# gmarcais/Jellyfish

Measured on AMD Instinct MI355X. Metric: k-mers/sec at k=21 canonical, 150 bp synthetic reads, bit-exact counts, higher is better.
Workload: dtype u64

## Files before the change

### jellyfish_amd/csrc/jfgpu.hip

```cpp
#include <hip/hip_runtime.h>
#include <math.h>
#include <stdint.h>
#include <stdio.h>
#include <string.h>
#include <algorithm>
#include <memory>
#include <string>
#include <type_traits>
#include <vector>

#include "../../include/jfgpu.h"
#include "gf2_matrix.hpp"
#include "tuning.hpp"
#include "kernels.hip.hpp"
#include "kernels_part.hip.hpp"
#include "kernels_tile.hip.hpp"
#include "kernels_p1ring.hip.hpp"
#include "kernels_bloom.hip.hpp"
#include "kernels_bloom_part.hip.hpp"
#include "kernels_wide.hip.hpp"
#include "kernels_wide_part.hip.hpp"
#include "kernels_nword.hip.hpp"
#include "kernels_parse.hip.hpp"
#include "kernels_bgzf.hip.hpp"
// ... 783 lines not shown
    HIP_TRY(hipFuncSetAttribute((const void*)tile_insert_wide_kernel<true>, hipFuncAttributeMaxDynamicSharedMemorySize, wt));
    HIP_TRY(hipFuncSetAttribute((const void*)tile_insert_wide_kernel<false>, hipFuncAttributeMaxDynamicSharedMemorySize, wt));
    HIP_TRY(hipFuncSetAttribute((const void*)tile_insert_wide_pipe_kernel<true>, hipFuncAttributeMaxDynamicSharedMemorySize, wt));
    HIP_TRY(hipFuncSetAttribute((const void*)tile_insert_wide_pipe_kernel<false>, hipFuncAttributeMaxDynamicSharedMemorySize, wt));
  }
  jfgpu_table* raw = t.release();
  int rc = jfgpu_clear(raw);
  if(rc) { jfgpu_destroy(raw); return rc; }
  *out = raw;
  return JFGPU_OK;
}

void jfgpu_destroy(jfgpu_table* t) {
  if(!t) return;
  hipSetDevice(t->device);
  if(t->stream) hipStreamSynchronize(t->stream);
  prof_collect(t);
  for(auto e : t->ev_pool) hipEventDestroy(e);
  hipFree(t->dt.slots); hipFree(t->d_fwd); hipFree(t->d_inv);
  if(t->d_dt) hipFree(t->d_dt);
  hipFree(t->dt.ovf_key); hipFree(t->dt.ovf_cnt); hipFree(t->dt.counters); hipFree(t->dt.dirty);
  for(int i = 0; i < 2; ++i) { if(t->d_stage[i]) hipFree(t->d_stage[i]); if(t->stage_done[i]) hipEventDestroy(t->stage_done[i]); }
  if(t->d_dump) hipFree(t->d_dump);
  if(t->d_bcache) hipFree(t->d_bcache);
  if(t->d_tile_off) hipFree(t->d_tile_off);
  part_discard(t);
  if(t->d_M1) hipFree(t->d_M1);
  if(t->d_strag) hipFree(t->d_strag);
  if(t->d_strag2) hipFree(t->d_strag2);
  if(t->d_strag2_n) hipFree(t->d_strag2_n);
  if(t->d_strag_n) hipFree(t->d_strag_n);
  if(t->d_M2) hipFree(t->d_M2);
  if(t->ws) hipFree(t->ws);
  if(t->stream2) hipStreamDestroy(t->stream2);
  for(auto ev : t->flush_ev) if(ev) hipEventDestroy(ev);
  if(t->flush_done) hipEventDestroy(t->flush_done);
  if(t->stream) hipStreamDestroy(t->stream);
  delete t;
}

int jfgpu_get_info(const jfgpu_table* t, jfgpu_info* o) {
  if(!t || !o) return fail(JFGPU_E_INVALID, "null argument");
  memset(o, 0, sizeof(*o));
  o->k = t->g.k; o->key_len = t->g.key_bits; o->canonical = t->g.canonical;
  o->lsize = t->g.lsize_g; o->size = 1ull << t->g.lsize_g; o->local_size = 1ull << t->g.lsize_l;
  o->shard_bits = t->g.shard_bits; o->shard_id = t->g.shard_id;
  o->val_len = t->g.cnt_bits; o->slot_bytes = (uint32_t)slot_bytes_of(t); o->tile_slots = 1u << t->g.tile_bits;
  o->matrix_identity = t->matrix.identity ? 1 : 0;
  o->out_counter_len = t->out_counter_len;
  o->max_reprobe = t->dt.max_probe;
  o->table_bytes = (1ull << t->g.lsize_l) * slot_bytes_of(t);
  return JFGPU_OK;
}

int jfgpu_get_matrix(const jfgpu_table* t, uint64_t* columns) {
  if(!t || !columns) return fail(JFGPU_E_INVALID, "null argument");
  memcpy(columns, t->matrix.columns.data(), sizeof(uint64_t) * t->matrix.c);
  return JFGPU_OK;
}

int jfgpu_clear(jfgpu_table* t) {
  if(t) { t->failed = 0; t->failed_msg.clear(); }
  int rc = use(t); if(rc) return rc;
  part_discard(t);
  HIP_TRY(hipMemsetAsync(t->dt.slots, 0, (1ull << t->g.lsize_l) * slot_bytes_of(t), t->stream));
  HIP_TRY(hipMemsetAsync(t->dt.ovf_key, 0, t->ovf_cap * sizeof(uint64_t), t->stream));
  HIP_TRY(hipMemsetAsync(t->dt.ovf_cnt, 0, t->ovf_cap * sizeof(uint64_t), t->stream));
  HIP_TRY(hipMemsetAsync(t->dt.counters, 0, CTR_COUNT * sizeof(uint64_t), t->stream));
  HIP_TRY(hipMemsetAsync(t->dt.dirty, 0, (size_t)1 << (t->g.lsize_l - t->g.tile_bits), t->stream));
  HIP_TRY(hipStreamSynchronize(t->stream));
  t->pristine = true; t->occ_known = 0; t->fed_since = 0; t->direct_seen = 0; t->occ_bound = 0; t->bigval_bound = 0; t->ovf_failed_need = 0;
  t->flushes_plain = 0; t->flushes_heavy = 0;
  t->n_p2_roles = t->n_p2_ring = t->n_p2_sort = t->n_p2_exact = t->n_p1_ring = t->n_p1_other = t->n_tile_dense = 0;
  return JFGPU_OK;
}

int jfgpu_sync(jfgpu_table* t) {
  int rc = use(t); if(rc) return rc;
  rc = part_flush(t); if(rc) return rc;
  HIP_TRY(hipStreamSynchronize(t->stream));
#ifdef JFGPU_PHASE_PROF
  { unsigned long long c[24], z[24] = {0};
    if(hipMemcpyFromSymbol(c, HIP_SYMBOL(g_phase_prof), sizeof c) == hipSuccess) {
      fprintf(stderr, "[phase prof] P1 (ring): stage %llu  encode+hash+append %llu  (barrier) %llu  units out %llu  finish %llu\n",
              c[0], c[1], c[2], c[3], c[4]);
      fprintf(stderr, "[phase prof] P2: (barrier) %llu  load %llu  hist %llu  scan %llu  lds-scatter %llu  write-out %llu  finish %llu\n",
              c[8], c[9], c[10], c[11], c[12], c[13], c[14]);
      fprintf(stderr, "[phase prof] T: loop+offsets %llu  rank adds + fill %llu  place %llu  merge %llu  queue (wave 0's own) %llu  (its wait for the others) %llu  store %llu\n",
              c[16], c[17], c[18], c[22], c[21], c[19], c[20]);
      (void)hipMemcpyToSymbol(HIP_SYMBOL(g_phase_prof), z, sizeof z);
    } }
#endif
#ifdef JFGPU_TILE_PROF
  { uint64_t c[CTR_COUNT]; if(read_counters(t, c) == JFGPU_OK)
      fprintf(stderr, "[tile prof] wait+prefetch %llu  fill %llu  insert %llu  store %llu (shader clocks, summed over blocks)\n",
              (unsigned long long)c[CTR_PROF0], (unsigned long long)c[CTR_PROF0 + 1], (unsigned long long)c[CTR_PROF0 + 2], (unsigned long long)c[CTR_PROF0 + 3]); }
#endif
  return check_deferred(t);
}

int jfgpu_wait(jfgpu_table* t) {
  int rc = use(t); if(rc) return rc;
  HIP_TRY(hipStreamSynchronize(t->stream));
  return JFGPU_OK;
}

int jfgpu_count_ascii_dev(jfgpu_table* t, const char* d_bases, size_t n) {
  int rc = use(t); if(rc) return rc;
  if(t->g.shard_bits) return fail(JFGPU_E_INVALID, "sharded table: count through its communicator (jfgpu_comm_count_ascii_dev)");
  if(!d_bases && n) return fail(JFGPU_E_INVALID, "null buffer");
  return launch_count(t, d_bases, n);
}

int jfgpu_count_ascii(jfgpu_table* t, const char* bases, size_t n) {
  int rc = use(t); if(rc) return rc;
  if(t->g.shard_bits) return fail(JFGPU_E_INVALID, "sharded table: count through its communicator (jfgpu_comm_count_ascii_dev)");
  if(!bases && n) return fail(JFGPU_E_INVALID, "null buffer");
  if(n < t->g.k) return JFGPU_OK;
  rc = ensure_stage(t); if(rc) return rc;
  const size_t step = kStageBytes - (t->g.k - 1);
  for(size_t o = 0; o < n; o += step) {
    const size_t len = std::min(kStageBytes, n - o);
    const int b = t->stage_next; t->stage_next ^= 1;
    HIP_TRY(hipEventSynchronize(t->stage_done[b]));
    HIP_TRY(hipMemcpyAsync(t->d_stage[b], bases + o, len, hipMemcpyHostToDevice, t->stream));
    rc = launch_count(t, (const char*)t->d_stage[b], len); if(rc) return rc;
    HIP_TRY(hipEventRecord(t->stage_done[b], t->stream));
    if(o + len >= n) break;
  }
  return JFGPU_OK;
}

static int add_keys_piece(jfgpu_table* t, const uint64_t* d_keys, size_t n, uint64_t val, uint8_t* d_is_new) {
  int rc = JFGPU_OK;
  if(!n) return JFGPU_OK;
  { const bool big = t->g.cnt_bits < 64 && (val >> t->g.cnt_bits) != 0;
    rc = ensure_ovf(t, big ? 0 : (uint64_t)n * val, big ? n : 0); if(rc) return rc; }
  const bool one_word = !t->wide && !t->nword;
  if(one_word && val == 1 && !d_is_new && use_partitioned(t, n * 8)) {
    const int prc = part_ingest(t, (const uint8_t*)d_keys, 0, (int64_t)n, true, n);
    if(prc >= 0) return prc;
  }
  if(one_word && (d_is_new || val != 1)) { rc = part_flush(t); if(rc) return rc; }
  if(!t->wide) t->pristine = false;
  const int grid = grid_for(t, (n + kBlock - 1) / kBlock);
  ProfScope ps(t, 1, n);
  if(one_word && val == 1 && !d_is_new) {
    if(t->returning) hipLaunchKernelGGL(add_keys_one_kernel<true>, dim3(grid), dim3(kBlock), 0, t->stream, t->dt, d_keys, (uint64_t)n);
    else             hipLaunchKernelGGL(add_keys_one_kernel<false>, dim3(grid), dim3(kBlock), 0, t->stream, t->dt, d_keys, (uint64_t)n);
  } else {
    with_view(t, [&](const auto& T) {
      hipLaunchKernelGGL(add_keys_kernel, dim3(grid), dim3(kBlock), 0, t->stream, T, d_keys, (uint64_t)n, t->key_words, val, d_is_new);
    });
  }
  HIP_TRY(hipGetLastError());
  return JFGPU_OK;
}

int jfgpu_add_keys_dev(jfgpu_table* t, const uint64_t* d_keys, size_t n, uint64_t val, uint8_t* d_is_new) {
  int rc = use(t); if(rc) return rc;
  if(!n) return JFGPU_OK;
  if(!d_keys) return fail(JFGPU_E_INVALID, "null keys");
  if(!capacity_managed(t)) return add_keys_piece(t, d_keys, n, val, d_is_new);
  size_t off = 0;
  while(off < n) {
    uint64_t take = 0;
    rc = ensure_capacity(t, n - off, &take); if(rc) return rc;
    rc = add_keys_piece(t, d_keys + off * t->key_words, (size_t)take, val, d_is_new ? d_is_new + off : nullptr); if(rc) return rc;
    off += (size_t)take;
  }
  return JFGPU_OK;
}

// ... 395 lines not shown
```

### jellyfish_amd/csrc/kernels.hip.hpp

```cpp
#pragma once
#include <hip/hip_runtime.h>
#include <stdint.h>
#include "kmer_core.hpp"

namespace jfgpu {

constexpr int kBlock = 256;
constexpr int kPerThread = kPerLane;
constexpr int kTilePos = kBlock * kPerThread;

enum Counter : int { CTR_FULL = 0, CTR_MERS = 1, CTR_OVF_FULL = 2, CTR_OVF_USED = 3, CTR_MISROUTED = 4, CTR_DIRECT = 5,
                     CTR_T_ITEMS = 6, CTR_T_QUEUED = 7 ,
                     CTR_PROF0 = 8 , CTR_COUNT = 12 };

#ifdef JFGPU_PHASE_PROF
__device__ unsigned long long g_phase_prof[24];
struct PhaseClk {
  long long acc[8] = {0, 0, 0, 0, 0, 0, 0, 0}; long long t;
  __device__ PhaseClk() { t = clock64(); }
  __device__ void mark(int i) { const long long n = clock64(); acc[i] += n - t; t = n; }
  __device__ void flush(int base) { if(threadIdx.x == 0) for(int i = 0; i < 8; ++i) if(acc[i]) atomicAdd(&g_phase_prof[base + i], (unsigned long long)acc[i]); }
};
#define JF_PHASE(pc, i) (pc).mark(i)
#define JF_PHASE_FLUSH(pc, base) (pc).flush(base)
#else
struct PhaseClk {};
#define JF_PHASE(pc, i) do {} while(0)
#define JF_PHASE_FLUSH(pc, base) do {} while(0)
#endif

struct DevBloom {
  uint32_t* data;
  uint64_t m;
  uint64_t recip;
  uint32_t nh;
  uint32_t nbytes;
  uint32_t kind;
  uint32_t pad_;
  const uint64_t* tbl1;
  const uint64_t* tbl2;
  uint64_t* cache;
  uint64_t cache_mask;
};

struct DevTable {
  TableGeom g;
  uint64_t* slots;
  const uint64_t* fwd_tbl;
  const uint64_t* inv_tbl;
  uint64_t* ovf_key;
  uint64_t* ovf_cnt;
  uint64_t ovf_mask;
  uint64_t* counters;
  uint32_t max_probe;
  DevBloom bloom;
  uint8_t* dirty;
};

#if defined(JFGPU_EMU)
__device__ __forceinline__ void lds_barrier() { __syncthreads(); }
#define JF_DYN_LDS(name) unsigned char* name = ::hip_emu::dyn_lds()
#else
__device__ __forceinline__ void lds_barrier() { asm volatile("s_waitcnt lgkmcnt(0)\n\ts_barrier" ::: "memory"); }
#define JF_DYN_LDS(name) extern __shared__ __align__(16) unsigned char name[]
#endif

__device__ inline bool bloom_admits(const DevBloom& B, uint64_t key);
__device__ inline uint32_t bloom_admit_mask(const DevBloom& B, const TableGeom& g, const LaneWords& L);

__device__ inline void ovf_add(const DevTable& T, uint64_t slot, uint64_t units) {
  const uint64_t want = slot + 1;
  uint64_t h = (slot * 0x9E3779B97F4A7C15ull) >> 20;
  for(uint64_t p = 0; p <= T.ovf_mask; ++p) {
    const uint64_t s = (h + p) & T.ovf_mask;
    unsigned long long old = atomicCAS((unsigned long long*)&T.ovf_key[s], 0ull, (unsigned long long)want);
    if(old == 0ull) atomicAdd((unsigned long long*)&T.counters[CTR_OVF_USED], 1ull);
    if(old == 0ull || old == want) {
      atomicAdd((unsigned long long*)&T.ovf_cnt[s], (unsigned long long)units);
      return;
    }
  }
  atomicAdd((unsigned long long*)&T.counters[CTR_OVF_FULL], 1ull);
}

__device__ inline uint64_t ovf_get(const DevTable& T, uint64_t slot) {
  const uint64_t want = slot + 1;
  uint64_t h = (slot * 0x9E3779B97F4A7C15ull) >> 20;
  for(uint64_t p = 0; p <= T.ovf_mask; ++p) {
    const uint64_t s = (h + p) & T.ovf_mask;
    const uint64_t k = T.ovf_key[s];
    if(k == 0) return 0;
    if(k == want) return T.ovf_cnt[s];
  }
  return 0;
}

__device__ inline uint64_t full_count(const DevTable& T, uint64_t word, uint64_t slot, bool have_ovf) {
  uint64_t c = slot_count(T.g, word);
  if(have_ovf) c += ovf_get(T, slot) << T.g.cnt_bits;
  return c;
}

__device__ __forceinline__ uint64_t slot_ld(const DevTable& T, uint64_t i) {
  return T.g.slot32 ? (uint64_t)reinterpret_cast<const uint32_t*>(T.slots)[i] : T.slots[i];
}
__device__ __forceinline__ uint64_t slot_ld_relaxed(const DevTable& T, uint64_t i) {
  if(T.g.slot32) return __hip_atomic_load(reinterpret_cast<const uint32_t*>(T.slots) + i, __ATOMIC_RELAXED, __HIP_MEMORY_SCOPE_AGENT);
  return __hip_atomic_load(&T.slots[i], __ATOMIC_RELAXED, __HIP_MEMORY_SCOPE_AGENT);
}
__device__ __forceinline__ uint64_t slot_cas(const DevTable& T, uint64_t i, uint64_t cmp, uint64_t val) {
  if(T.g.slot32) return atomicCAS(reinterpret_cast<unsigned int*>(T.slots) + i, (unsigned int)cmp, (unsigned int)val);
// ... 765 lines not shown
```

### jellyfish_amd/csrc/kernels_p1ring.hip.hpp

```cpp
#pragma once
#include <type_traits>
#include "kernels_part.hip.hpp"

namespace jfgpu {

template <int P> __device__ __forceinline__ void wave_prio() {
#if defined(__HIP_DEVICE_COMPILE__)
  __builtin_amdgcn_s_setprio(P);
#endif
}

__device__ __forceinline__ uint32_t adm_to_vmask(uint32_t adm) {
  uint32_t r = 0;
#pragma unroll
  for(int j = 0; j < 16; ++j) r |= ((adm >> j) & 1u) << (15 - j);
  return r;
}


constexpr uint32_t kStragPerBlock = 16384;

template <typename ITEM, uint32_t RB = 128> struct Ring {
  static constexpr uint32_t kSlots = RB / sizeof(ITEM);
  static constexpr uint32_t kUnit = 64 / sizeof(ITEM);
  static constexpr uint32_t kChunk = 16 / sizeof(ITEM);
  static constexpr uint32_t kFull = 0xFFFFu & ~(kSlots - 1);
  static constexpr uint32_t kWords = sizeof(ITEM) <= 4 ? 1 : 1 + sizeof(ITEM) / 8;
  __device__ static uint32_t first_fill(uint32_t b) { return ((kChunk * b) & (kSlots - 1)) << 16; }
};

template <typename ITEM> __device__ __forceinline__ uint32_t chunk_hole_key(const uint4& v) {
  if constexpr(sizeof(ITEM) == 4) { const uint32_t a = v.x > v.y ? v.x : v.y, c = v.z > v.w ? v.z : v.w; return a > c ? a : c; }
  else if constexpr(sizeof(ITEM) == 8) { const uint32_t a = v.x & v.y, c = v.z & v.w; return a > c ? a : c; }
  else return v.x & v.y & v.z & v.w;
}
template <typename ITEM, typename F> __device__ __forceinline__ void chunk_items(const uint4& v, F&& f) {
  if constexpr(sizeof(ITEM) == 4) { f((ITEM)v.x); f((ITEM)v.y); f((ITEM)v.z); f((ITEM)v.w); }
  else if constexpr(sizeof(ITEM) == 8) { f((ITEM)(((uint64_t)v.y << 32) | v.x)); f((ITEM)(((uint64_t)v.w << 32) | v.z)); }
  else f((ITEM)(((unsigned __int128)(((uint64_t)v.w << 32) | v.z) << 64) | (((uint64_t)v.y << 32) | v.x)));
}

template <typename ITEM> __device__ __forceinline__ void strag_store(uint64_t* rec, uint32_t b, ITEM item, uint32_t cnt) {
  const uint64_t meta = ((uint64_t)(cnt < 255u ? cnt : 255u) << 56) | ((uint64_t)(b & 0xFFFFFFu) << 32);
  if constexpr(sizeof(ITEM) == 4) rec[0] = meta | (uint32_t)item;
  else if constexpr(sizeof(ITEM) == 8) { rec[0] = meta; rec[1] = (uint64_t)item; }
  else { rec[0] = meta; rec[1] = (uint64_t)item; rec[2] = (uint64_t)(item >> 64); }
}
template <typename ITEM> __device__ __forceinline__ void strag_load(const uint64_t* rec, uint32_t& b, ITEM& item, uint32_t& cnt) {
  const uint64_t meta = rec[0];
  b = (uint32_t)(meta >> 32) & 0xFFFFFFu; cnt = (uint32_t)(meta >> 56);
  if constexpr(sizeof(ITEM) == 4) item = (ITEM)(uint32_t)meta;
  else if constexpr(sizeof(ITEM) == 8) item = (ITEM)rec[1];
  else item = (ITEM)(((unsigned __int128)rec[2] << 64) | rec[1]);
}

struct RingBooks { uint32_t gpos = 0, room = 0, nxt = 0, stored = 0; bool nxt_asked = false, exhausted = false; };

template <typename ITEM, bool OWNED = false, uint32_t RB = 128, typename STRAG>
__device__ __forceinline__ void ring_flush(ITEM* s_ring, uint32_t* s_fill, uint32_t t, bool all, RingBooks& B, ITEM* my_region, uint32_t cap,
                                           unsigned int* gcur, unsigned int* gshort, STRAG&& straggler) {
  using R = Ring<ITEM, RB>;
  const ITEM hole = (ITEM)~(ITEM)0;
  const uint32_t w = s_fill[t];
  uint32_t cnt = w & 0xFFFFu; if(cnt > R::kSlots) cnt = R::kSlots;
  const uint32_t rb = (w >> 16) & (R::kSlots - 1);
  uint32_t units = cnt / R::kUnit; if(all && (cnt % R::kUnit)) ++units;
  uint32_t nout = 0;
  for(uint32_t s = 0; s < units; ++s) {
    uint4 v[4];
    const uint32_t s0 = (rb + s * R::kUnit) & (R::kSlots - 1);
#pragma unroll
    for(int q = 0; q < 4; ++q) v[q] = *reinterpret_cast<const uint4*>(s_ring + t * R::kSlots + ((s0 + R::kChunk * q) & (R::kSlots - 1)));
    if(!all) {
      uint32_t mx = 0;
#pragma unroll
      for(int q = 0; q < 4; ++q) { const uint32_t a = chunk_hole_key<ITEM>(v[q]); mx = mx > a ? mx : a; }
      if(mx == 0xFFFFFFFFu) break;
    }
    if constexpr(!OWNED) {
    if(B.room == 0 && B.nxt_asked) {
      if((uint64_t)B.nxt + kGran <= cap) { B.gpos = B.nxt; B.room = kGran; }
      else { B.exhausted = true; if(B.nxt < cap) atomicMax(&gshort[t], cap - B.nxt); }
      B.nxt_asked = false;
    }
    if(B.room == 0 && !B.exhausted) {
      const uint32_t r0 = atomicAdd(&gcur[t], kGran);
      if((uint64_t)r0 + kGran <= cap) { B.gpos = r0; B.room = kGran; }
      else { B.exhausted = true; if(r0 < cap) atomicMax(&gshort[t], cap - r0); }
    }
    }
    if(B.room) {
      uint4* dst = reinterpret_cast<uint4*>(my_region + B.gpos);
#pragma unroll
      for(int q = 0; q < 4; ++q) dst[q] = v[q];
      const uint32_t real = cnt - s * R::kUnit < R::kUnit ? cnt - s * R::kUnit : R::kUnit;
      B.gpos += OWNED ? real : R::kUnit; B.room -= R::kUnit; B.stored += real;
    } else {
#pragma unroll
      for(int q = 0; q < 4; ++q) chunk_items<ITEM>(v[q], [&](ITEM x) { if(x != hole) straggler(t, x, 1u); });
    }
#pragma unroll
    for(int q = 0; q < 4; ++q)
      *reinterpret_cast<uint4*>(s_ring + t * R::kSlots + ((s0 + R::kChunk * q) & (R::kSlots - 1))) = make_uint4(0xFFFFFFFFu, 0xFFFFFFFFu, 0xFFFFFFFFu, 0xFFFFFFFFu);
    ++nout;
  }
  if constexpr(!OWNED) { if(!all && !B.nxt_asked && !B.exhausted && B.room < R::kSlots) { B.nxt = atomicAdd(&gcur[t], kGran); B.nxt_asked = true; } }
  uint32_t expect = w;
  while(nout || (expect & 0xFFFFu) > R::kSlots) {
    uint32_t c = expect & 0xFFFFu; if(c > R::kSlots) c = R::kSlots;
    const uint32_t taken = nout * R::kUnit < c ? nout * R::kUnit : c;
    const uint32_t neww = ((((expect >> 16) + nout * R::kUnit) & 0xFFFFu) << 16) | (c - taken);
    const uint32_t old = atomicCAS(&s_fill[t], expect, neww);
    if(old == expect) break;
    expect = old;
  }
}

template <typename ITEM, uint32_t RB = 128>
__device__ __forceinline__ void ring_init(ITEM* s_ring, uint32_t* s_fill, uint32_t nb, uint32_t* s_nstrag) {
  using R = Ring<ITEM, RB>;
  for(uint32_t j = threadIdx.x; j < nb; j += blockDim.x) s_fill[j] = R::first_fill(j);
  uint4* r4 = reinterpret_cast<uint4*>(s_ring);
  for(uint32_t j = threadIdx.x; j < nb * (RB / 16) + RB / 16; j += blockDim.x) r4[j] = make_uint4(0xFFFFFFFFu, 0xFFFFFFFFu, 0xFFFFFFFFu, 0xFFFFFFFFu);
  if(threadIdx.x == 0) *s_nstrag = 0;
}

template <typename ITEM>
__device__ __forceinline__ void ring_finish(const RingBooks& B, uint32_t t, ITEM* my_region, uint32_t cap, unsigned int* gshort, unsigned long long* tot) {
  const ITEM hole = (ITEM)~(ITEM)0;
  for(uint32_t r = 0; r < B.room; ++r) my_region[B.gpos + r] = hole;
  if(B.nxt_asked) {
    if((uint64_t)B.nxt + kGran <= cap) { for(uint32_t r = 0; r < kGran; ++r) my_region[B.nxt + r] = hole; }
    else if(B.nxt < cap) atomicMax(&gshort[t], cap - B.nxt);
  }
  if(tot && B.stored) atomicAdd(&tot[t], (unsigned long long)B.stored);
}

struct OneWordDirect {
  static constexpr bool kCountsDirect = true;
  const DevTable* Tm; uint32_t b2; int returning;
  __device__ void operator()(uint32_t b, uint64_t item, uint32_t cnt) const { item_direct_call(Tm, b2, b, item, cnt, returning); }
};
struct RouteListDirect {
  static constexpr bool kCountsDirect = false;
  StragList SL;
  __device__ void operator()(uint32_t b, uint64_t item, uint32_t cnt) const {
    for(uint32_t i = 0; i < cnt; ++i) { const unsigned long long at = atomicAdd(SL.n, 1ull); if(at < SL.cap) SL.rec[at] = ((uint64_t)b << 32) | (uint32_t)item; }
  }
};

template <typename ITEM, bool BLOOM, int NB, int CANON, typename DIRECT = OneWordDirect>
__global__ __launch_bounds__(kPBlock) void p1_ring_kernel(DevTable T, DIRECT D, PartGeom P, const uint8_t* __restrict__ base,
                                                          int64_t lo, int64_t hi, uint32_t cap,
                                                          unsigned int* __restrict__ gcur,
                                                          unsigned long long* __restrict__ tot,
                                                          ITEM* __restrict__ out,
                                                          uint64_t* __restrict__ strag, uint32_t* __restrict__ strag_n) {
  using R = Ring<ITEM>;
  constexpr int RP = sizeof(ITEM) == 4 ? 8 : 4;
  JF_DYN_LDS(s_dyn);
  ITEM* s_ring = reinterpret_cast<ITEM*>(s_dyn);
  __shared__ uint64_t s_fwd[NB < 0 ? 1 : 8 * 256];
  __shared__ uint32_t s_fill[kGranMaxB + 32];
  __shared__ uint32_t s_nstrag;
  __shared__ uint32_t s_codes[kPBlock + 2];
  __shared__ uint32_t s_inv[kPBlock + 2];
  const TableGeom& g = T.g;
  const uint32_t nb = 1u << P.b1;
  const uint32_t t = threadIdx.x, lane = t & 63;
  const bool owner = t < nb;
  const ITEM hole = (ITEM)~(ITEM)0;
  if constexpr(NB >= 0) load_tables_lds(s_fwd, T.fwd_tbl, g.nbytes);
  ring_init<ITEM>(s_ring, s_fill, nb, &s_nstrag);
  const uint32_t dump = nb * R::kSlots + (lane & (R::kSlots - 1));
  [[maybe_unused]] const uint32_t xs_hi_mask = g.lsize_g > 32 ? (g.lsize_g >= 64 ? 0xFFFFFFFFu : ((1u << (g.lsize_g - 32)) - 1u)) : 0u;
  unsigned int* const gshort = gcur + nb;
  uint64_t* const my_strag = strag + (size_t)blockIdx.x * kStragPerBlock * R::kWords;
  const uint32_t k = g.k, bshift = g.lsize_l - P.b1;
  const uint32_t rc_shift = 2 * (k - 1);
  const uint32_t rest_mask = P.rest_shift >= 32 ? 0xFFFFFFFFu : ((1u << P.rest_shift) - 1u);
  RingBooks B;
  if(owner) { B.nxt = atomicAdd(&gcur[t], kGran); B.nxt_asked = true; }
  ITEM* const my_region = out + (uint64_t)t * cap;
  uint32_t my_mers = 0, my_direct = 0;

  auto straggler = [&](uint32_t b, ITEM item, uint32_t cnt) {
    const uint32_t at = atomicAdd(&s_nstrag, 1u);
    if(at < kStragPerBlock) strag_store<ITEM>(my_strag + (size_t)at * R::kWords, b, item, cnt);
    else { D(b, (uint64_t)item, cnt); ++my_direct; }
  };

  const int64_t n_tiles = (hi + kPTilePos - 1) / kPTilePos;
  TileRaw Rw = tile_fetch(base, (int64_t)blockIdx.x * kPTilePos, lo, hi);
  lds_barrier();
  [[maybe_unused]] PhaseClk pc;
  for(int64_t tile = blockIdx.x; tile < n_tiles; tile += gridDim.x) {
    const LaneWords L = tile_stage(Rw, tile * kPTilePos, lo, hi, s_codes, s_inv);
    Rw = tile_fetch(base, (tile + gridDim.x) * kPTilePos, lo, hi);
    JF_PHASE(pc, 0);
    const uint32_t adm = BLOOM ? bloom_admit_mask(T.bloom, g, L) : 0xFFFFu;
    uint64_t fw = (((uint64_t)L.p2 << 32) | L.p1) & g.key_mask;
    uint64_t rc = revcomp64(fw, k);
    uint64_t smear = L.inv48;
    for(uint32_t s = 1; s < k; ) { const uint32_t step = s < k - s ? s : k - s; smear |= smear >> step; s += step; }
    const uint32_t rawmask = ~(uint32_t)smear & 0xFFFFu;
    const uint32_t vmask = BLOOM ? (rawmask & adm_to_vmask(adm)) : rawmask;
    my_mers += (uint32_t)__popc(rawmask);
    auto rounds = [&](auto runs_tag) {
    constexpr bool RUNS = decltype(runs_tag)::value;
    uint64_t pk = 0; uint32_t pv = 0, run = 0;
#pragma unroll 1
    for(int j0 = 0; j0 < kPerLane; j0 += RP) {
      constexpr int NE = RUNS ? RP + 1 : RP;
      uint32_t ea[NE], eo[NE]; ITEM ei[NE];
      [[maybe_unused]] uint32_t spm = 0;
#pragma unroll
      for(int e = 0; e < NE; ++e) { ea[e] = dump; ei[e] = 0; eo[e] = 0; }
      auto emit = [&](int e, uint64_t key, uint32_t cnt, bool on) {
        uint32_t b; ITEM item;
        if constexpr(NB == kHashXS && sizeof(ITEM) == 4) {
          uint32_t ylo, yhi;
          xs_hash_halves<false>((uint32_t)key, (uint32_t)(key >> 32), xs_hi_mask, ylo, yhi);
          b = funnel_r(yhi, ylo, bshift) & (nb - 1);
          item = ((ylo & rest_mask) << g.rem_bits) | ((uint32_t)(key >> 32) >> (g.lsize_g - 32));
        } else {
          const uint64_t pos = NB < 0 ? xs_hash(key, g.lsize_g, g.key_bits) : hash_tables_t<(NB < 0 ? 0 : NB)>(s_fwd, key, g.nbytes);
          b = (uint32_t)(pos >> bshift) & (nb - 1);
          if constexpr(sizeof(ITEM) == 4) item = (((uint32_t)pos & rest_mask) << g.rem_bits) | (uint32_t)(key >> g.lsize_g);
          else item = make_item<ITEM>(g, P, key, pos & g.local_mask);
        }
        const bool special = on && (item == hole || cnt > 1);
        const bool normal = on && !special;
#ifndef JFGPU_P1_LATE_SPECIAL
        if(special) straggler(b, item, cnt);
        const uint32_t o = atomicAdd(&s_fill[normal ? b : nb + (lane & 31u)], 1u);
        ea[e] = normal ? b * R::kSlots : dump; ei[e] = item; eo[e] = normal ? o : 0u;
#else
        const uint32_t o = atomicAdd(&s_fill[normal ? b : nb + (lane & 31u)], 1u);
        spm |= special ? 1u << e : 0u;
        ea[e] = on ? b * R::kSlots : dump; ei[e] = item; eo[e] = normal ? o : special ? (R::kFull | ((cnt < 0xFFFFu ? cnt : 0xFFFFu) << 16)) : 0u;
#endif
      };
#ifndef JFGPU_P1_OLD_EXTRACT
      const uint32_t cur_r = L.cur << (2 * j0), ncur_r = ~cur_r, vm_r = vmask << j0;
#endif
#pragma unroll
      for(int e = 0; e < RP; ++e) {
#ifndef JFGPU_P1_OLD_EXTRACT
        const uint32_t c = (cur_r >> (2 * (15 - e))) & 3u, nc = (ncur_r >> (2 * (15 - e))) & 3u;
        const uint32_t v = vm_r & (1u << (15 - e));
#else
        const int j = j0 + e;
        const uint32_t c = (L.cur >> (2 * (15 - j))) & 3u, nc = 3u - c;
        const uint32_t v = vmask & (1u << (15 - j));
#endif
        if constexpr(NB >= 5 || NB == kHashXS) {
          const uint32_t flo = (uint32_t)fw, fhi = (uint32_t)(fw >> 32), rlo = (uint32_t)rc, rhi = (uint32_t)(rc >> 32);
          fw = ((uint64_t)(funnel_r(fhi, flo, 30) & (uint32_t)(g.key_mask >> 32)) << 32) | ((flo << 2) | c);
          rc = ((uint64_t)((rhi >> 2) | (nc << (rc_shift - 32))) << 32) | funnel_r(rhi, rlo, 2);
        } else {
          fw = ((fw << 2) | c) & g.key_mask;
          rc = (rc >> 2) | ((uint64_t)nc << rc_shift);
        }
        const uint64_t key = ((CANON == 1 || (CANON == 2 && g.canonical)) && rc < fw) ? rc : fw;
        if constexpr(RUNS) {
#ifdef JFGPU_P1_NO_RUNS
          const bool same = false;
#else
          const bool same = v && pv && key == pk;
#endif
          emit(e, pk, run, pv && !same);
          run = same ? run + 1 : 1;
          pk = key; pv = v;
        } else emit(e, key, 1u, v != 0);
      }
      if constexpr(RUNS) { if(j0 + RP >= kPerLane) { emit(NE - 1, pk, run, pv != 0); pv = 0; } }
      uint32_t ghosts = 0;
#pragma unroll
      for(int e = 0; e < NE; ++e) {
        const uint32_t full = eo[e] & R::kFull;
        ghosts |= full;
        const uint32_t at = ea[e] + ((eo[e] + (eo[e] >> 16)) & (R::kSlots - 1));
        s_ring[full ? dump : at] = ei[e];
      }
      if(ghosts) {
#pragma unroll 1
#ifndef JFGPU_P1_LATE_SPECIAL
        for(int e = 0; e < NE; ++e) {
          uint32_t a = 0, o = 0; ITEM it = 0;
#pragma unroll
          for(int q = 0; q < NE; ++q) if(q == e) { a = ea[q]; o = eo[q]; it = ei[q]; }
          if(o & R::kFull) straggler(a / R::kSlots, it, 1u);
        }
#else
        for(int e = 0; e < NE; ++e) if(eo[e] & R::kFull) straggler(ea[e] / R::kSlots, ei[e], ((spm >> e) & 1u) ? eo[e] >> 16 : 1u);
#endif
      }
      JF_PHASE(pc, 1);
      lds_barrier();
      JF_PHASE(pc, 2);
#ifndef JFGPU_P1_NO_FLUSH_PRIO
      wave_prio<3>();
#endif
      if(owner) ring_flush<ITEM>(s_ring, s_fill, t, false, B, my_region, cap, gcur, gshort, straggler);
#ifndef JFGPU_P1_NO_FLUSH_PRIO
      wave_prio<0>();
#endif
      JF_PHASE(pc, 3);
    }
    };
    bool may_run = k < 14;
    {
      const uint32_t hc = L.cur ^ (L.cur >> 2), hp = L.p1 ^ (L.p1 >> 2);
      may_run = may_run || (hc & 0x3FFFu) == 0 || ((hc >> 16) & 0x3FFFu) == 0 || (hp & 0x3FFFu) == 0;
    }
#ifdef JFGPU_P1_ALWAYS_RUNS
    may_run = true;
#endif
    if(__ballot(may_run) != 0ull) rounds(std::true_type{}); else rounds(std::false_type{});
  }
  lds_barrier();
  if(owner) { ring_flush<ITEM>(s_ring, s_fill, t, true, B, my_region, cap, gcur, gshort, straggler); ring_finish<ITEM>(B, t, my_region, cap, gshort, tot); }
  lds_barrier();
  if(t == 0) strag_n[blockIdx.x] = s_nstrag < kStragPerBlock ? s_nstrag : kStragPerBlock;
  JF_PHASE(pc, 4);
  JF_PHASE_FLUSH(pc, 0);
  if(DIRECT::kCountsDirect && my_direct) atomicAdd((unsigned long long*)&T.counters[CTR_DIRECT], (unsigned long long)my_direct);
  uint64_t w = my_mers;
  for(int o = 32; o > 0; o >>= 1) w += __shfl_down(w, o, 64);
  if((threadIdx.x & 63) == 0 && w) atomicAdd((unsigned long long*)&T.counters[CTR_MERS], (unsigned long long)w);
}

template <typename ITEM, typename DIRECT>
__global__ __launch_bounds__(256) void p1_stragglers_kernel(DIRECT D, unsigned long long* __restrict__ ctr_direct, const uint64_t* __restrict__ strag,
                                                            const uint32_t* __restrict__ strag_n, uint32_t n_lists, uint32_t cap,
                                                            unsigned int* __restrict__ gcur, unsigned long long* __restrict__ tot,
                                                            ITEM* __restrict__ out, uint32_t list_cap = kStragPerBlock) {
  using R = Ring<ITEM>;
  uint32_t my_direct = 0;
  for(uint32_t l = blockIdx.x; l < n_lists; l += gridDim.x) {
    const uint32_t n = strag_n[l];
    const uint64_t* rec = strag + (size_t)l * list_cap * R::kWords;
    for(uint32_t i = threadIdx.x; i < n; i += blockDim.x) {
      uint32_t b, cnt; ITEM item;
      strag_load<ITEM>(rec + (size_t)i * R::kWords, b, item, cnt);
      if(cnt == 1 && item != (ITEM)~(ITEM)0) {
        const uint32_t at = atomicAdd(&gcur[b], 1u);
        if(at < cap) { out[(uint64_t)b * cap + at] = item; if(tot) atomicAdd(&tot[b], 1ull); continue; }
        atomicMin(&gcur[b], cap);
      }
      D(b, item, cnt);
      ++my_direct;
    }
  }
  if(ctr_direct && my_direct) atomicAdd(ctr_direct, (unsigned long long)my_direct);
}

constexpr uint32_t kP2StragPerBlock = 2048;

struct P2RingDirect {
  const DevTable* Tm; uint32_t b2; uint32_t dest_shift; int returning;
  __device__ void operator()(uint32_t dest, uint64_t item, uint32_t cnt) const { item_direct_call(Tm, b2, dest >> dest_shift, item, cnt, returning); }
};

template <typename DIRECT>
__global__ __launch_bounds__(kPBlock) void p2_ring_kernel(DIRECT D, uint32_t b2e, uint32_t tag_bits, SegList S, uint32_t cap,
                                                          unsigned int* __restrict__ gcur, unsigned int* __restrict__ gshort,
                                                          uint32_t* __restrict__ out, uint32_t bucket0, unsigned long long* __restrict__ tot,
                                                          uint64_t* __restrict__ strag, uint32_t* __restrict__ strag_n, unsigned long long* __restrict__ ctr_direct) {
  using R = Ring<uint32_t>;
  constexpr int RP = 8;
  JF_DYN_LDS(s_dyn);
  uint32_t* s_ring = reinterpret_cast<uint32_t*>(s_dyn);
  __shared__ uint32_t s_fill[kGranMaxB];
  __shared__ uint32_t s_nstrag;
  const uint32_t nb = 1u << b2e;
  const uint32_t bucket = bucket0 + blockIdx.y;
  const uint32_t dest0 = bucket * nb;
  const uint32_t t = threadIdx.x, lane = t & 63;
  const bool owner = t < nb;
  const uint32_t hole = 0xFFFFFFFFu;
  ring_init<uint32_t>(s_ring, s_fill, nb, &s_nstrag);
  const uint32_t dump = nb * R::kSlots + (lane & (R::kSlots - 1));
  unsigned int* const gc = gcur + dest0;
  unsigned int* const gs = gshort + dest0;
  const uint32_t list = blockIdx.y * gridDim.x + blockIdx.x;
  uint64_t* const my_strag = strag + (size_t)list * kP2StragPerBlock;
  RingBooks B;
  if(owner) { B.nxt = atomicAdd(&gc[t], kGran); B.nxt_asked = true; }
  uint32_t* const my_region = out + ((uint64_t)dest0 + t) * cap;
  uint32_t my_direct = 0;
  auto straggler = [&](uint32_t d, uint32_t item, uint32_t cnt) {
    const uint32_t at = atomicAdd(&s_nstrag, 1u);
    if(at < kP2StragPerBlock) strag_store<uint32_t>(my_strag + at, dest0 + d, item, cnt);
    else { D(dest0 + d, (uint64_t)item, cnt); ++my_direct; }
  };
  auto flush = [&](bool all) { if(owner) ring_flush<uint32_t>(s_ring, s_fill, t, all, B, my_region, cap, gc, gs, straggler); };
  lds_barrier();
  uint32_t seg = 0; uint64_t my_a = 0, my_b = 0;
  const uint32_t* src = nullptr;
  auto next_seg = [&]() -> bool {
    for(; seg < S.n; ++seg) {
      const uint64_t a0 = seg_lo(S, seg, bucket), b0 = seg_hi(S, seg, bucket);
      const uint64_t len4 = (b0 - a0 + 3) / 4;
      const uint64_t per4 = (len4 + gridDim.x - 1) / gridDim.x;
      const uint64_t q0 = (uint64_t)blockIdx.x * per4, q1 = q0 + per4;
      const uint64_t e1 = a0 + 4 * (q1 < len4 ? q1 : len4);
      my_a = a0 + 4 * (q0 < len4 ? q0 : len4); my_b = e1 < b0 ? e1 : b0;
      src = reinterpret_cast<const uint32_t*>(S.items[seg]);
      if(my_a < my_b) return true;
    }
    return false;
  };
// ... 212 lines not shown
```

Measured before the change: 15.63 billion.

## Split P1 ring block into two staggered halves to overlap flush with sweep

Rewrites the P1 ring kernel main loop so the block works as two half-blocks offset by half a round. Each half loads and publishes its own input half-tile, and the ring flush (service) of one half runs while the other half sweeps. The goal is to hide the per-round barrier and flush latency that previously stalled the whole block. It also adds optional profiling counters for ghosts and straggler entries. Each half now covers only half the positions per tile, so the ring slots may fill faster and produce more stragglers. The new path is enabled by default for non-bloom 4-byte items.

```diff
diff --git a/jellyfish_amd/csrc/jfgpu.hip b/jellyfish_amd/csrc/jfgpu.hip
--- a/jellyfish_amd/csrc/jfgpu.hip
+++ b/jellyfish_amd/csrc/jfgpu.hip
@@ -889,13 +889,25 @@
 #ifdef JFGPU_PHASE_PROF
   { unsigned long long c[24], z[24] = {0};
     if(hipMemcpyFromSymbol(c, HIP_SYMBOL(g_phase_prof), sizeof c) == hipSuccess) {
+#if JFGPU_P1_HALVES
+      fprintf(stderr, "[phase prof] P1 (ring, halves): A sweep %llu  (its barrier) %llu  service %llu  (its barrier) %llu | B sweep %llu  (its barrier) %llu  service %llu  (its barrier) %llu\n",
+              c[0], c[1], c[2], c[3], c[4], c[5], c[6], c[7]);
+#else
       fprintf(stderr, "[phase prof] P1 (ring): stage %llu  encode+hash+append %llu  (barrier) %llu  units out %llu  finish %llu\n",
               c[0], c[1], c[2], c[3], c[4]);
+#endif
       fprintf(stderr, "[phase prof] P2: (barrier) %llu  load %llu  hist %llu  scan %llu  lds-scatter %llu  write-out %llu  finish %llu\n",
               c[8], c[9], c[10], c[11], c[12], c[13], c[14]);
       fprintf(stderr, "[phase prof] T: loop+offsets %llu  rank adds + fill %llu  place %llu  merge %llu  queue (wave 0's own) %llu  (its wait for the others) %llu  store %llu\n",
               c[16], c[17], c[18], c[22], c[21], c[19], c[20]);
       (void)hipMemcpyToSymbol(HIP_SYMBOL(g_phase_prof), z, sizeof z);
+    } }
+#endif
+#if defined(JFGPU_PHASE_PROF) || defined(JFGPU_P1_RING_COUNTS)
+  { unsigned long long r[2], rz[2] = {0, 0};
+    if(hipMemcpyFromSymbol(r, HIP_SYMBOL(g_p1_ring_prof), sizeof r) == hipSuccess) {
+      fprintf(stderr, "[phase prof] P1 (ring): ghosts %llu  straggler-list entries %llu\n", r[0], r[1]);
+      (void)hipMemcpyToSymbol(HIP_SYMBOL(g_p1_ring_prof), rz, sizeof rz);
     } }
 #endif
 #ifdef JFGPU_TILE_PROF
diff --git a/jellyfish_amd/csrc/kernels.hip.hpp b/jellyfish_amd/csrc/kernels.hip.hpp
--- a/jellyfish_amd/csrc/kernels.hip.hpp
+++ b/jellyfish_amd/csrc/kernels.hip.hpp
@@ -23,10 +23,20 @@
 };
 #define JF_PHASE(pc, i) (pc).mark(i)
 #define JF_PHASE_FLUSH(pc, base) (pc).flush(base)
+#define JF_PHASE_FLUSH_AT(pc, base, lane) do { if(threadIdx.x == (lane)) for(int i_ = 0; i_ < 8; ++i_) if((pc).acc[i_]) atomicAdd(&g_phase_prof[(base) + i_], (unsigned long long)(pc).acc[i_]); } while(0)
 #else
 struct PhaseClk {};
 #define JF_PHASE(pc, i) do {} while(0)
 #define JF_PHASE_FLUSH(pc, base) do {} while(0)
+#define JF_PHASE_FLUSH_AT(pc, base, lane) do {} while(0)
+#endif
+#if defined(JFGPU_PHASE_PROF) || defined(JFGPU_P1_RING_COUNTS)
+__device__ unsigned long long g_p1_ring_prof[2];
+#define JF_P1_RING_COUNT(slot, n) atomicAdd(&g_p1_ring_prof[slot], (unsigned long long)(n))
+#define JF_P1_RING_TALLY(x) (++(x))
+#else
+#define JF_P1_RING_COUNT(slot, n) do {} while(0)
+#define JF_P1_RING_TALLY(x) do {} while(0)
 #endif
 
 struct DevBloom {
diff --git a/jellyfish_amd/csrc/kernels_p1ring.hip.hpp b/jellyfish_amd/csrc/kernels_p1ring.hip.hpp
--- a/jellyfish_amd/csrc/kernels_p1ring.hip.hpp
+++ b/jellyfish_amd/csrc/kernels_p1ring.hip.hpp
@@ -7,6 +7,14 @@
 template <int P> __device__ __forceinline__ void wave_prio() {
 #if defined(__HIP_DEVICE_COMPILE__)
   __builtin_amdgcn_s_setprio(P);
+#endif
+}
+
+__device__ __forceinline__ uint32_t wave_uniform(uint32_t x) {
+#if defined(__HIP_DEVICE_COMPILE__)
+  return __builtin_amdgcn_readfirstlane(x);
+#else
+  return x;
 #endif
 }
 
@@ -148,6 +156,38 @@
     for(uint32_t i = 0; i < cnt; ++i) { const unsigned long long at = atomicAdd(SL.n, 1ull); if(at < SL.cap) SL.rec[at] = ((uint64_t)b << 32) | (uint32_t)item; }
   }
 };
+
+#ifndef JFGPU_P1_HALVES
+#define JFGPU_P1_HALVES 1
+#endif
+constexpr uint32_t kPHalf = kPBlock / 2;
+constexpr int64_t kPHalfPos = (int64_t)kPHalf * kPerLane;
+
+__device__ inline TileRaw half_fetch(const uint8_t* __restrict__ base, int64_t start, uint32_t l, int64_t lo, int64_t hi) {
+  TileRaw R;
+  raw16(base, start + 16 * (int64_t)l, lo, hi, R.w);
+  R.h[0] = R.h[1] = R.h[2] = R.h[3] = 0;
+  if(l < 2) raw16(base, start - 32 + 16 * (int64_t)l, lo, hi, R.h);
+  return R;
+}
+__device__ inline void half_publish(const TileRaw& R, int64_t start, uint32_t l, int64_t lo, int64_t hi, uint32_t* codes, uint32_t* inv) {
+  uint32_t c, v;
+  edges16(R.w, start + 16 * (int64_t)l, lo, hi, c, v);
+  codes[l + 2] = c; inv[l + 2] = v;
+  if(l < 2) {
+    uint32_t hc, hv;
+    edges16(R.h, start - 32 + 16 * (int64_t)l, lo, hi, hc, hv);
+    codes[l] = hc; inv[l] = hv;
+  }
+}
+__device__ inline LaneWords half_words(const uint32_t* codes, const uint32_t* inv, uint32_t l) {
+  LaneWords L;
+  L.cur = codes[l + 2];
+  L.p1 = codes[l + 1];
+  L.p2 = codes[l];
+  L.inv48 = ((uint64_t)inv[l] << 32) | ((uint64_t)inv[l + 1] << 16) | inv[l + 2];
+  return L;
+}
 
 template <typename ITEM, bool BLOOM, int NB, int CANON, typename DIRECT = OneWordDirect>
 __global__ __launch_bounds__(kPBlock) void p1_ring_kernel(DevTable T, DIRECT D, PartGeom P, const uint8_t* __restrict__ base,
@@ -163,8 +203,9 @@
   __shared__ uint64_t s_fwd[NB < 0 ? 1 : 8 * 256];
   __shared__ uint32_t s_fill[kGranMaxB + 32];
   __shared__ uint32_t s_nstrag;
-  __shared__ uint32_t s_codes[kPBlock + 2];
-  __shared__ uint32_t s_inv[kPBlock + 2];
+  constexpr bool HALVES = JFGPU_P1_HALVES && !BLOOM && sizeof(ITEM) == 4;
+  __shared__ uint32_t s_codes[kPBlock + 4];
+  __shared__ uint32_t s_inv[kPBlock + 4];
   const TableGeom& g = T.g;
   const uint32_t nb = 1u << P.b1;
   const uint32_t t = threadIdx.x, lane = t & 63;
@@ -183,6 +224,7 @@
   if(owner) { B.nxt = atomicAdd(&gcur[t], kGran); B.nxt_asked = true; }
   ITEM* const my_region = out + (uint64_t)t * cap;
   uint32_t my_mers = 0, my_direct = 0;
+  [[maybe_unused]] uint32_t my_ghosts = 0;
 
   auto straggler = [&](uint32_t b, ITEM item, uint32_t cnt) {
     const uint32_t at = atomicAdd(&s_nstrag, 1u);
@@ -191,13 +233,8 @@
   };
 
   const int64_t n_tiles = (hi + kPTilePos - 1) / kPTilePos;
-  TileRaw Rw = tile_fetch(base, (int64_t)blockIdx.x * kPTilePos, lo, hi);
-  lds_barrier();
   [[maybe_unused]] PhaseClk pc;
-  for(int64_t tile = blockIdx.x; tile < n_tiles; tile += gridDim.x) {
-    const LaneWords L = tile_stage(Rw, tile * kPTilePos, lo, hi, s_codes, s_inv);
-    Rw = tile_fetch(base, (tile + gridDim.x) * kPTilePos, lo, hi);
-    JF_PHASE(pc, 0);
+  auto work_tile = [&](const LaneWords& L, auto&& round_end) {
     const uint32_t adm = BLOOM ? bloom_admit_mask(T.bloom, g, L) : 0xFFFFu;
     uint64_t fw = (((uint64_t)L.p2 << 32) | L.p1) & g.key_mask;
     uint64_t rc = revcomp64(fw, k);
@@ -290,23 +327,13 @@
           uint32_t a = 0, o = 0; ITEM it = 0;
 #pragma unroll
           for(int q = 0; q < NE; ++q) if(q == e) { a = ea[q]; o = eo[q]; it = ei[q]; }
-          if(o & R::kFull) straggler(a / R::kSlots, it, 1u);
+          if(o & R::kFull) { straggler(a / R::kSlots, it, 1u); JF_P1_RING_TALLY(my_ghosts); }
         }
 #else
         for(int e = 0; e < NE; ++e) if(eo[e] & R::kFull) straggler(ea[e] / R::kSlots, ei[e], ((spm >> e) & 1u) ? eo[e] >> 16 : 1u);
 #endif
       }
-      JF_PHASE(pc, 1);
-      lds_barrier();
-      JF_PHASE(pc, 2);
-#ifndef JFGPU_P1_NO_FLUSH_PRIO
-      wave_prio<3>();
-#endif
-      if(owner) ring_flush<ITEM>(s_ring, s_fill, t, false, B, my_region, cap, gcur, gshort, straggler);
-#ifndef JFGPU_P1_NO_FLUSH_PRIO
-      wave_prio<0>();
-#endif
-      JF_PHASE(pc, 3);
+      round_end(j0);
     }
     };
     bool may_run = k < 14;
@@ -318,17 +345,85 @@
     may_run = true;
 #endif
     if(__ballot(may_run) != 0ull) rounds(std::true_type{}); else rounds(std::false_type{});
+  };
+  auto flush_due = [&]() {
+#ifndef JFGPU_P1_NO_FLUSH_PRIO
+    wave_prio<3>();
+#endif
+    if(owner) ring_flush<ITEM>(s_ring, s_fill, t, false, B, my_region, cap, gcur, gshort, straggler);
+#ifndef JFGPU_P1_NO_FLUSH_PRIO
+    wave_prio<0>();
+#endif
+  };
+  if constexpr(!HALVES) {
+    TileRaw Rw = tile_fetch(base, (int64_t)blockIdx.x * kPTilePos, lo, hi);
+    lds_barrier();
+    for(int64_t tile = blockIdx.x; tile < n_tiles; tile += gridDim.x) {
+      const LaneWords L = tile_stage(Rw, tile * kPTilePos, lo, hi, s_codes, s_inv);
+      Rw = tile_fetch(base, (tile + gridDim.x) * kPTilePos, lo, hi);
+      JF_PHASE(pc, 0);
+      work_tile(L, [&](int) {
+        JF_PHASE(pc, 1);
+        lds_barrier();
+        JF_PHASE(pc, 2);
+        flush_due();
+        JF_PHASE(pc, 3);
+      });
+    }
+  } else {
+    const bool half_a = wave_uniform(t) < kPHalf;
+    const uint32_t hl = t & (kPHalf - 1);
+    uint32_t* const h_codes = s_codes + (half_a ? 0u : kPHalf + 2);
+    uint32_t* const h_inv = s_inv + (half_a ? 0u : kPHalf + 2);
+    const int64_t hoff = half_a ? 0 : kPHalfPos;
+    int64_t pub = blockIdx.x;
+    TileRaw Rw = half_fetch(base, pub * kPTilePos + hoff, hl, lo, hi);
+    if(half_a) {
+      half_publish(Rw, pub * kPTilePos + hoff, hl, lo, hi, h_codes, h_inv);
+      pub += gridDim.x;
+      Rw = half_fetch(base, pub * kPTilePos + hoff, hl, lo, hi);
+    }
+    lds_barrier();
+    JF_PHASE(pc, 3);
+    auto service = [&](bool publish) __attribute__((always_inline)) {
+      flush_due();
+      if(publish) {
+        half_publish(Rw, pub * kPTilePos + hoff, hl, lo, hi, h_codes, h_inv);
+        pub += gridDim.x;
+        Rw = half_fetch(base, pub * kPTilePos + hoff, hl, lo, hi);
+      }
+      JF_PHASE(pc, 2);
+      lds_barrier();
+      JF_PHASE(pc, 3);
+    };
+    auto round_end = [&](int j0) {
+      const bool last = j0 + RP >= kPerLane;
+      JF_PHASE(pc, 0);
+      lds_barrier();
+      JF_PHASE(pc, 1);
+      if(half_a || !last) service(half_a && last);
+    };
+    for(int64_t pair = blockIdx.x; pair < n_tiles; pair += gridDim.x) {
+      if(!half_a) service(true);
+      const LaneWords L = half_words(h_codes, h_inv, hl);
+      work_tile(L, round_end);
+    }
   }
   lds_barrier();
   if(owner) { ring_flush<ITEM>(s_ring, s_fill, t, true, B, my_region, cap, gcur, gshort, straggler); ring_finish<ITEM>(B, t, my_region, cap, gshort, tot); }
   lds_barrier();
-  if(t == 0) strag_n[blockIdx.x] = s_nstrag < kStragPerBlock ? s_nstrag : kStragPerBlock;
-  JF_PHASE(pc, 4);
-  JF_PHASE_FLUSH(pc, 0);
+  if(t == 0) { strag_n[blockIdx.x] = s_nstrag < kStragPerBlock ? s_nstrag : kStragPerBlock; JF_P1_RING_COUNT(1, s_nstrag < kStragPerBlock ? s_nstrag : kStragPerBlock); }
+  if constexpr(!HALVES) { JF_PHASE(pc, 4); JF_PHASE_FLUSH(pc, 0); }
+  else { JF_PHASE_FLUSH_AT(pc, 0, 0); JF_PHASE_FLUSH_AT(pc, 4, kPHalf); }
   if(DIRECT::kCountsDirect && my_direct) atomicAdd((unsigned long long*)&T.counters[CTR_DIRECT], (unsigned long long)my_direct);
   uint64_t w = my_mers;
   for(int o = 32; o > 0; o >>= 1) w += __shfl_down(w, o, 64);
   if((threadIdx.x & 63) == 0 && w) atomicAdd((unsigned long long*)&T.counters[CTR_MERS], (unsigned long long)w);
+#if defined(JFGPU_PHASE_PROF) || defined(JFGPU_P1_RING_COUNTS)
+  uint64_t gh = my_ghosts;
+  for(int o = 32; o > 0; o >>= 1) gh += __shfl_down(gh, o, 64);
+  if((threadIdx.x & 63) == 0 && gh) JF_P1_RING_COUNT(0, gh);
+#endif
 }
 
 template <typename ITEM, typename DIRECT>
```

Measured after the change: 15.60 billion. Within noise of the previous version (-0.1%).
